# ChristianFeldmann/libHM

Hardware: AMD Instinct MI355X
Metric: decoded Mpixels/s (luma), 2160p Main10 reconstruction + loop filters (higher is better)
Workload: dtype int16 samples / int32 accumulate; 1 GPU; 3840x2160 Main10 lowdelay_P pictures, pre-parsed CTU metadata: prep+MC+dequant/IT/recon+deblock+SAO, batch of 16 independent pictures per step, inputs resident in HBM; sub_benchmark=full, streams=2, parallelism=frame-parallel, 1 process per GPU, no data-path collective

## Files before the change

libhm_amd/csrc/hmgpu_api.hip:

```cpp
#include "hmgpu_host.h"

#include <algorithm>
#include <cstdio>
#include <cstring>
#include <cstdlib>
#include <new>
#include <vector>

namespace hmgpu_host __attribute__((visibility("hidden"))) {

hipError_t h2d_small(hmgpu_ctx* c, void* dst, const void* src, size_t bytes, hipStream_t hs) {
  const size_t need = (bytes + 63) & ~(size_t)63;
  if (!c->bounce || need > hmgpu_ctx::kBounceSeg) return hipMemcpyAsync(dst, src, bytes, hipMemcpyHostToDevice, hs);
  if (c->bounce_off + need > hmgpu_ctx::kBounceSeg) {
    hipStream_t streams[3] = {c->stream, c->copy_stream, c->copy_stream2};
    for (int k = 0; k < 3; k++) (void)hipEventRecord(c->bounce_ev[c->bounce_seg][k], streams[k]);
    c->bounce_used[c->bounce_seg] = true;
    c->bounce_seg = (c->bounce_seg + 1) % hmgpu_ctx::kBounceSegs;
    c->bounce_off = 0;
    if (c->bounce_used[c->bounce_seg]) for (int k = 0; k < 3; k++) (void)hipEventSynchronize(c->bounce_ev[c->bounce_seg][k]);
  }
  char* at = c->bounce + (size_t)c->bounce_seg * hmgpu_ctx::kBounceSeg + c->bounce_off;
  memcpy(at, src, bytes);
  c->bounce_off += need;
// ... 224 lines not shown
  if (c->fmt != 1) {
    for (int i = 0; i < b.n; i++) {
      const PicDev& d = c->pics[b.pic[i]].dev;
      HIP_TRY(c, hipMemsetAsync(d.resid[1], 0, (size_t)((char*)d.resid[2] - (char*)d.resid[1]) + c->coef_elems[2] * sizeof(int16_t), c->stream));
    }
  }
  McArgs ma;
  memset(&ma, 0, sizeof(ma));
  ma.n = b.n; ma.width = c->seq.width; ma.height = c->seq.height; ma.log2ctu = c->seq.log2_ctu_size; ma.ctus_w = c->ctus_w;
  ma.tw = c->grid_w / 2; ma.npics = c->seq.max_pictures;
  ma.slab = c->plane_slab; ma.pic_stride = 2 * c->plane_bytes; ma.slab_bytes = ma.pic_stride * c->pics.size(); ma.sao_off = (uint32_t)c->plane_bytes;
  for (size_t i = 0; i < c->pics.size(); i++)
    if (c->pics[i].sao_applied) (i < 32 ? ma.sao_mask_lo : ma.sao_mask_hi) |= 1u << (i & 31);
  for (int i = 0; i < b.n; i++) {
    const PicDev& d = c->pics[b.pic[i]].dev;
    ma.first_ctu[i] = b.first_ctu[i]; ma.num_ctus[i] = b.num_ctus[i];
    ma.tmv[i] = d.tmv; ma.slices[i] = d.slices;
  }
  const PicDev& d0 = c->pics[b.pic[0]].dev;
  const char* const base0 = (const char*)c->pics[b.pic[0]].planes;
  uint32_t bps = (uint32_t)std::max(4, std::min(b.n >= 4 ? 12 : 24, max_ctus / 8 + 1));
  {
    ItxArgs ia;
    memset(&ia, 0, sizeof(ia));
    ia.n = b.n; ia.class_mask = 0xf;
    for (int k = 0; k < 3; k++) { ia.rtw[k] = (c->grid_w / 2) >> (k ? c->csx : 0); ia.bd[k] = d0.bd[k]; }
    ia.csx = c->csx; ia.csy = c->csy;
    for (int k = 0; k < 4; k++) ia.tu_cap[k] = c->tu_cap[k];
    for (int i = 0; i < b.n; i++) {
      const PicDev& d = c->pics[b.pic[i]].dev;
      for (int k = 0; k < 4; k++) ia.tu[i][k] = d.tu[k];
      ia.tu_count[i] = d.tu_count;
      for (int k = 0; k < 3; k++) { ia.coef[i][k] = d.coef[k]; ia.resid[i][k] = d.resid[k]; }
      ia.sl_m[i] = d.sl_m;
    }
    ProfScope ps(c, K_ITX);
    launch_itx(ia, bps, c->stream);
    bool any_ccp = false;
    for (int i = 0; i < b.n; i++) any_ccp |= c->pics[b.pic[i]].dev.ccp[0] != nullptr;
    if (any_ccp) launch_ccp(c->d_pics, b, max_ctus, c->stream);
  }
  {
    ProfScope ps(c, K_MC_LUMA);
    ma.pitch = c->pitch[0]; ma.bd = c->seq.bit_depth_luma;
    ma.origin_off = (uint32_t)((const char*)d0.rec[0] - base0);
    ma.rtw = c->grid_w / 2;
    for (int i = 0; i < b.n; i++) { ma.dst[i] = c->pics[b.pic[i]].dev.rec[0]; ma.resid[i] = c->pics[b.pic[i]].dev.resid[0]; }
    launch_mc_luma(ma, max_ctus, any_wp, any_bi, c->stream);
    if (any_cells) { ProfScope pc(c, K_MC_CELLS); launch_mc_luma_cells(c->d_pics, c->d_finals, b, max_ctus, c->seq.log2_ctu_size, any_wp, c->stream); }
  }
  if (c->fmt != 1) {
    ProfScope ps(c, K_MC_CHROMA);
    launch_mc_chroma_fmt(c->d_pics, c->d_finals, b, max_ctus, c->seq.log2_ctu_size, c->fmt, any_wp, c->stream);
  } else if (c->seq.chroma_format != 0) {
    ProfScope ps(c, K_MC_CHROMA);
    ma.pitch = c->pitch[1]; ma.bd = c->seq.bit_depth_chroma;
    ma.origin_off = (uint32_t)((const char*)d0.rec[1] - base0);
    ma.cr_off = 0;
    ma.rtw = c->grid_w / 4;
    for (int i = 0; i < b.n; i++) {
      const PicDev& d = c->pics[b.pic[i]].dev;
      ma.dst[i] = d.rec[1]; ma.dst2[i] = d.rec[2]; ma.resid[i] = d.resid[1]; ma.resid2[i] = d.resid[2];
    }
    launch_mc_chroma(ma, max_ctus, any_wp, any_bi, c->stream);
    if (any_cells) { ProfScope pc(c, K_MC_CELLS); launch_mc_chroma_cells(c->d_pics, c->d_finals, b, max_ctus, c->seq.log2_ctu_size, any_wp, c->stream); }
  }
  if (any_intra) {
    ProfScope ps(c, K_INTRA);
    launch_intra(c->d_pics, b, c->d_ctu_order, c->num_ctus, !any_islice, c->stream);
    if (c->fmt == 2) launch_intra_chroma_422(c->d_pics, b, c->stream);
    for (int i = 0; i < b.n; i++) if (std::find(c->intra_launched.begin(), c->intra_launched.end(), b.pic[i]) == c->intra_launched.end()) c->intra_launched.push_back(b.pic[i]);
  }
  HIP_TRY(c, hipGetLastError());
  return HMGPU_OK;
}

hmgpu_status run_filter(hmgpu_ctx* c, const Batch& b, int stages) {
// ... 129 lines not shown
  c->grid_w = c->ctus_w * c->pw; c->grid_h = c->ctus_h * c->pw;
  c->fmt = seq->chroma_format == 0 ? 1 : seq->chroma_format;
  c->csx = c->fmt == 3 ? 0 : 1; c->csy = c->fmt == 1 ? 1 : 0;
  c->mx[0] = 128; c->mx[1] = c->mx[2] = 128 >> c->csx;
  c->my[0] = 80; c->my[1] = c->my[2] = 80 >> c->csy;
  c->pitch[0] = (int)align_up((size_t)seq->width, 64) + 2 * c->mx[0] + 64;
  c->pitch[1] = c->pitch[2] = kCStep * ((int)align_up((size_t)seq->width >> c->csx, 64) + 2 * c->mx[1] + 64);
  c->rows[0] = c->ctus_h * c->ctu + 2 * c->my[0] + 8; c->rows[1] = c->rows[2] = ((c->ctus_h * c->ctu) >> c->csy) + 2 * c->my[1] + 8;
  c->coef_elems[0] = (size_t)c->num_ctus * c->ctu * c->ctu;
  c->coef_elems[1] = c->coef_elems[2] = c->coef_elems[0] >> (c->csx + c->csy);
  {
    const size_t blocks = ((size_t)c->num_ctus * (c->parts / 4) + 255) / 256;
    const size_t per_shard = (blocks + kTuShards - 1) / kTuShards;
    const uint32_t per_block[4] = {4 * 384, 4 * 96, 4 * 24, 4 * 4};
    for (int k = 0; k < 4; k++) c->tu_cap[k] = (uint32_t)(per_shard * (c->fmt == 1 ? per_block[k] : 3u * (1024u >> (2 * k))));
  }
  c->pics.resize(seq->max_pictures);
  c->h_finals.resize(seq->max_pictures);
  hmgpu_status st = HMGPU_OK;
  c->plane_bytes = plane_set_bytes(c);
  if (hipMalloc((void**)&c->plane_slab, c->plane_bytes * 2 * seq->max_pictures) != hipSuccess ||
      hipMemset(c->plane_slab, 0, c->plane_bytes * 2 * seq->max_pictures) != hipSuccess) st = HMGPU_EDEVICE;
  for (int i = 0; i < seq->max_pictures && st == HMGPU_OK; i++) st = alloc_picture(c, c->pics[i]);
  if (st == HMGPU_OK) {
    {
      std::vector<int32_t> order;
      for (int d = 0; d <= 2 * (c->ctus_h - 1) + c->ctus_w - 1; d++)
        for (int r = 0; r < c->ctus_h; r++) { const int col = d - 2 * r; if (col >= 0 && col < c->ctus_w) order.push_back(r * c->ctus_w + col); }
      if (hipMalloc((void**)&c->d_ctu_order, order.size() * sizeof(int32_t)) != hipSuccess ||
          hipMemcpy(c->d_ctu_order, order.data(), order.size() * sizeof(int32_t), hipMemcpyHostToDevice) != hipSuccess) st = HMGPU_EDEVICE;
// ... 429 lines not shown
```

libhm_amd/csrc/hmgpu_dev.h:

```cpp
#pragma once
#include <hip/hip_runtime.h>
#include <stdint.h>
#include "../../include/hmgpu.h"

namespace hmgpu {

constexpr int kMaxBatch = 16;
constexpr int kMaxPics = 64;
constexpr int kTuShards = 8;
constexpr int kCStep = 2;

struct __attribute__((aligned(16))) BlkInfo {
  int16_t mv[2][2];
  int8_t  ref[2];
  int8_t  qp;
  uint8_t flags;
  uint8_t edge;
  uint8_t log2cu;
  uint16_t slice;
};
static_assert(sizeof(BlkInfo) == 16, "BlkInfo must be 16 bytes");

enum : uint8_t {
  BF_VALID = 1,
// ... 105 lines not shown
  int32_t fmt, csx, csy;
  const int8_t* ccp[2];
  uint8_t* ctu_intra;
  uint32_t* intra_done;
  uint32_t* fault;
  int32_t debug_skip_ctu;
};

struct Batch {
  int32_t n;
  int32_t pic[kMaxBatch];
  int32_t first_ctu[kMaxBatch];
  int32_t num_ctus[kMaxBatch];
};

struct McArgs {
  int32_t n, mode, log2n, per;
  int32_t width, height, log2ctu, ctus_w;
  int32_t tw, pitch, bd, npics;
  int32_t first_ctu[kMaxBatch], num_ctus[kMaxBatch];
  const TileMv* tmv[kMaxBatch];
  int16_t* dst[kMaxBatch];
  int16_t* dst2[kMaxBatch];
  const int16_t* resid[kMaxBatch];
  const int16_t* resid2[kMaxBatch];
  int32_t rtw, pad_;
  const SliceDev* slices[kMaxBatch];
  const char* slab;
  uint64_t pic_stride, slab_bytes;
  uint32_t sao_off, origin_off, cr_off;
  uint32_t sao_mask_lo, sao_mask_hi;
};

struct ItxArgs {
  int32_t n; uint32_t class_mask;
  int32_t blocks[4];
  int32_t rtw[3], bd[3];
  int32_t csx, csy;
  uint32_t tu_cap[4];
  const TuRec* tu[kMaxBatch][4];
  const uint32_t* tu_count[kMaxBatch];
  const int16_t* coef[kMaxBatch][3];
  int16_t* resid[kMaxBatch][3];
  const uint8_t* sl_m[kMaxBatch];
};

#define HMGPU_AS1 __attribute__((address_space(1)))
// ... 204 lines not shown
```

libhm_amd/csrc/k_itx.hip:

```cpp
#include "hmgpu_dev.h"
#include "itx_core.h"
#include <algorithm>

namespace hmgpu {

template <int LOG2N> struct ItxLds {
  static constexpr int BYTES = PkCfg<LOG2N>::TPB * PkCfg<LOG2N>::TU_ELEMS * 2;
};
constexpr int kItxLdsBytes = std::max(std::max(ItxLds<2>::BYTES, ItxLds<3>::BYTES), std::max(ItxLds<4>::BYTES, ItxLds<5>::BYTES));

struct ItxPic {
  const TuRec* list; uint32_t count_cap; const uint32_t* count;
  const int16_t* coef[3]; int16_t* resid[3]; int32_t rtw[3], bd[3]; const uint8_t* sl_m;
  int32_t csx, csy;
};
template <typename T> __device__ inline T by_comp(const T (&v)[3], int comp) { return comp == 0 ? v[0] : comp == 1 ? v[1] : v[2]; }

template <int LOG2N>
__device__ inline void itx_class(const ItxPic& P, int bx, int nbx, char* __restrict__ lds_raw) {
  constexpr int N = 1 << LOG2N;
  const TuRec* __restrict__ list = P.list;
  const uint32_t cap = P.count_cap;
  const int j = threadIdx.x / N, n = threadIdx.x % N;
  int16_t* buf = reinterpret_cast<int16_t*>(lds_raw) + j * PkCfg<LOG2N>::TU_ELEMS;
  constexpr int TPW = 64 / N;
  const int jw = (threadIdx.x & 63) / N;
  const uint32_t stride = (uint32_t)nbx * 4 * TPW;
  uint32_t t = ((uint32_t)bx * 4 + (threadIdx.x >> 6)) * TPW + jw;
  struct Rec { uint32_t w0, w1, w2; };
  auto load_rec = [&](uint32_t ti, Rec& r) {
    r.w0 = r.w1 = r.w2 = 0;
    if (ti < cap) { const uint32_t* rp = reinterpret_cast<const uint32_t*>(list + ti); r.w0 = ldg(rp); r.w1 = ldg(rp + 1); r.w2 = ldg(rp + 2); }
  };
  Rec rc, rn;
  load_rec(t, rc);
  load_rec(t + stride, rn);
  const uint32_t count = min(ldg(P.count), cap);
  auto load_levels = [&](uint32_t ti, const Rec& r, uint32_t (&lv)[N / 2]) {
#pragma unroll
    for (int i = 0; i < N / 2; i++) lv[i] = 0;
    if (ti < count) {
      const int16_t* lev = by_comp(P.coef, r.w1 & 3) + r.w2 + n * N;
      if constexpr (N == 4) { const u32x2 a = ldg2(lev); lv[0] = a.x; lv[1] = a.y; }
      else {
#pragma unroll
        for (int i = 0; i < N / 8; i++) { const u32x4 a = ldg4(lev + i * 8); lv[4 * i] = a.x; lv[4 * i + 1] = a.y; lv[4 * i + 2] = a.z; lv[4 * i + 3] = a.w; }
      }
// ... 114 lines not shown
```

libhm_amd/csrc/k_mc.hip:

```cpp
#include "mc_core.h"
#include "itx_core.h"
#include <type_traits>

namespace hmgpu {

typedef u32x4 u32x4_a4 __attribute__((aligned(4)));
#if defined(MC_EXP) && (MC_EXP & 1)
__device__ inline u32x4 ldg4_a4(const void* p) { const uint32_t v = (uint32_t)(uintptr_t)p; return u32x4{v, v + 1, v + 2, v + 3}; }
#elif defined(MC_NT)
__device__ inline u32x4 ldg4_a4(const void* p) { return __builtin_nontemporal_load((const u32x4_a4 HMGPU_AS1*)p); }
#else
__device__ inline u32x4 ldg4_a4(const void* p) { return *(const u32x4_a4 HMGPU_AS1*)p; }
#endif
#ifndef MC_LB_LUMA
#define MC_LB_LUMA 7
#endif
#ifndef MC_LB_CHROMA
#define MC_LB_CHROMA 8
#endif

__device__ inline uint32_t pk_sub(uint32_t a, uint32_t b) {
  return __builtin_bit_cast(uint32_t, __builtin_bit_cast(short2v, a) - __builtin_bit_cast(short2v, b));
}

// ... 48 lines not shown
  asm("v_ashrrev_i32_sdwa %0, %1, %2 dst_sel:WORD_1 dst_unused:UNUSED_PRESERVE src0_sel:DWORD src1_sel:DWORD" : "+v"(d) : "v"(sh), "v"(hi));
  return d;
}

template <bool CHROMA> struct McLds {
  static constexpr int ROW_DW = CHROMA ? 128 : 256;
  struct { uint32_t body[2 * ROW_DW], halo[2 * ROW_DW]; } w[4];
  uint32_t taps[144];
  uint32_t htap[CHROMA ? 36 : 1];
#ifdef MC_LDS_PAD
  uint32_t pad[MC_LDS_PAD / 4];
#endif
};

struct Square { int sx, sy, ext; };
__device__ inline bool square_of_block(const McArgs& a, int& slot, Square& g) {
  int lb;
  if (a.mode) { slot = blockIdx.x & (a.n - 1); lb = (int)(blockIdx.x >> a.log2n) * a.per + (int)blockIdx.y; }
  else { slot = blockIdx.x; lb = blockIdx.y; }
  if (lb >= a.num_ctus[slot]) return false;
  const int ctu = a.first_ctu[slot] + lb, ctu_sz = 1 << a.log2ctu;
  g.sx = (ctu % a.ctus_w) * ctu_sz; g.sy = (ctu / a.ctus_w) * ctu_sz; g.ext = min(ctu_sz, 64);
  return true;
}

struct WpTile { bool active; int w0, o0, w1, o1, log2wd; };
template <bool WP>
__device__ inline WpTile wp_tile(const SliceDev* __restrict__ slices, uint32_t flags, uint32_t wpw, int comp) {
  WpTile w = {false, 1, 0, 1, 0, 0};
  if constexpr (WP) {
    const SliceDev& sd = slices[wpw >> 16];
    w.active = ldg(&sd.weighted_pred) != 0;
    if (w.active) {
      w.log2wd = ldg(&sd.wp_log2_denom[comp ? 1 : 0]);
      const int l0 = (flags & TM_FIRST_L1) ? 1 : 0, r0 = wpw & 15, r1 = (wpw >> 4) & 15;
      w.w0 = ldg(&sd.wp_weight[l0][r0][comp]); w.o0 = ldg(&sd.wp_offset[l0][r0][comp]);
      if (flags & TM_BI) { w.w1 = ldg(&sd.wp_weight[1][r1][comp]); w.o1 = ldg(&sd.wp_offset[1][r1][comp]); }
// ... 62 lines not shown
      const auto sw = __builtin_amdgcn_permlane32_swap(res[0][j], res[1][j], false, false);
      o[2 * j] = __builtin_amdgcn_perm(sw[1], sw[0], 0x05040100u);
      o[2 * j + 1] = __builtin_amdgcn_perm(sw[1], sw[0], 0x07060302u);
    }
    stg4(dst, u32x4{o[0], o[1], o[2], o[3]});
    return;
  }
#pragma unroll
  for (int r = 0; r < 2; r++) {
    int16_t* row = dst + (ptrdiff_t)r * pitch;
    if constexpr (W == 8) { u32x4 v = {res[r][0], res[r][1], res[r][2], res[r][3]}; stg4(row, v); }
    else { u32x2 v = {res[r][0], res[r][1]}; stg2(row, v); }
  }
}

__device__ inline u32x4 load_tile_rec(const McArgs& a, int slot, const Square& g, int x, int y) {
  const bool tin = x < g.sx + g.ext && y < g.sy + g.ext && x < a.width && y < a.height;
  u32x4 tm = {0, 0, 0, 0};
  if (tin) tm = ldg4(a.tmv[slot] + (size_t)(y >> 3) * a.tw + (x >> 3));
  return tm;
}
__device__ inline bool tile_is_top(const u32x4 tm, int r, int partner_lane) {
  const uint32_t u0 = __shfl((int)tm.x, partner_lane), u1 = __shfl((int)tm.y, partner_lane), u2 = __shfl((int)tm.z, partner_lane);
  return r == 0 || !(u0 == tm.x && u1 == tm.y && u2 == tm.z);
}

constexpr uint32_t kWinLimit = 0xffff0000u;
constexpr uint32_t kResidLimit = 0x7fffff00u;
template <bool BUF> struct Win;
template <> struct Win<true> {
  typedef uint32_t ref;
  __amdgpu_buffer_rsrc_t rs;
  uint32_t stride;
  __device__ inline Win(const McArgs& a, int) : rs(__builtin_amdgcn_make_buffer_rsrc((void*)a.slab, 0, kWinLimit, 0x00020000)), stride((uint32_t)a.pic_stride) {}
  __device__ inline ref nowhere() const { return kWinLimit; }
  __device__ inline ref plane(const McArgs& a, int pic) const {
    const uint32_t m = pic & 32 ? a.sao_mask_hi : a.sao_mask_lo;
    return (uint32_t)pic * stride + (__builtin_amdgcn_ubfe(m, (uint32_t)pic & 31u, 1u) ? a.sao_off : 0u) + a.origin_off;
  }
  __device__ inline ref at(ref pl, int row, int pitch, int x) const { return pl + (uint32_t)((row * pitch + x) * 2); }
  __device__ inline u32x4 load(ref o) const { return __builtin_bit_cast(u32x4, __builtin_amdgcn_raw_buffer_load_b128(rs, o, 0, 0)); }
};
template <> struct Win<false> {
  typedef const char* ref;
  const char* dummy;
  __device__ inline Win(const McArgs& a, int slot) : dummy(reinterpret_cast<const char*>(a.tmv[slot])) {}
  __device__ inline ref nowhere() const { return dummy; }
  __device__ inline ref plane(const McArgs& a, int pic) const {
    const uint32_t m = pic & 32 ? a.sao_mask_hi : a.sao_mask_lo;
    return a.slab + (size_t)(uint32_t)pic * a.pic_stride + (__builtin_amdgcn_ubfe(m, (uint32_t)pic & 31u, 1u) ? a.sao_off : 0u) + a.origin_off;
  }
  __device__ inline ref at(ref pl, int row, int pitch, int x) const { return pl + ((ptrdiff_t)row * pitch + x) * 2; }
  __device__ inline u32x4 load(ref p) const { return ldg4_a4(p); }
};

__device__ inline uint32_t from_right(uint32_t own, uint32_t first, bool take) {
  const uint32_t t = (uint32_t)__builtin_amdgcn_update_dpp(0, (int)first, 0x101, 0xf, 0xf, true);
  return take ? t : own;
}
__device__ inline u32x4 from_right(const u32x4 own, const u32x4 first, bool take) {
  return u32x4{from_right(own.x, first.x, take), from_right(own.y, first.y, take), from_right(own.z, first.z, take), from_right(own.w, first.w, take)};
}

__device__ inline void h_item_luma(const u32x4 (&r)[4], const uint32_t* __restrict__ tap, int sh1, uint32_t* __restrict__ out) {
// ... 34 lines not shown
__device__ inline uint32_t low_half(uint32_t v, int lane) { return (uint32_t)__shfl((int)v, lane & 31); }
__device__ inline const char* low_half(const char* p, int lane) {
  const uint64_t v = (uint64_t)(uintptr_t)p;
  return (const char*)(uintptr_t)(((uint64_t)low_half((uint32_t)(v >> 32), lane) << 32) | low_half((uint32_t)v, lane));
}

#ifndef MC_NO_F0
#define MC_F0 1
#endif
#ifndef MC_NO_R15
#define MC_R15 1
#endif
template <bool WP, bool BI, bool BUF>
__global__ void __launch_bounds__(256, (WP || BI) ? 1 : MC_LB_LUMA) k_mc_luma(const McArgs a) {
  __shared__ __attribute__((aligned(16))) McLds<false> S;
  int slot; Square g;
  if (!square_of_block(a, slot, g)) return;
  const int tid = threadIdx.x, lane = tid & 63, wave = tid >> 6;
  if (wave * 16 >= g.ext) return;
  const int pitch = a.pitch, bd = a.bd;
  const int tx = lane & 7, q = (lane >> 3) & 3, r = lane >> 5;
  const int x0 = g.sx + tx * 8, y0 = g.sy + wave * 16 + r * 8;
  const u32x4 tm = load_tile_rec(a, slot, g, x0, y0);
  if (lane < 36) *reinterpret_cast<u32x4*>(&S.taps[4 * lane]) = ldg4(&g_taps_luma.e[0][0] + 4 * lane);
  const uint32_t flags = tm.z >> 24, rmask = (tm.w >> 8) & 0xff;
  const bool active = (flags & TM_ACTIVE) != 0;
  if (!__ballot(active)) return;
#if defined(MC_EXP) && (MC_EXP & 64)
  bool top = tile_is_top(tm, r, lane ^ 32);
  if (wave > 0) {
    const u32x4 up = load_tile_rec(a, slot, g, x0, y0 - 8);
    if (r == 0 && up.x == tm.x && up.y == tm.y && up.z == tm.z) top = false;
  }
#else
  const bool top = tile_is_top(tm, r, lane ^ 32);
#endif
#ifdef MC_DEDUP
  const bool same_right = tx < 7 && !tile_is_top(tm, 1, lane + 1);
#else
  const bool same_right = false;
#endif
  const bool any_bi = BI && __ballot((flags & TM_BI) != 0) != 0;
  wave_lds_sync();
#ifdef MC_LDS_PAD
  if (a.n < 0) S.pad[tid] = 1;
#endif
  const int npass = any_bi ? 2 : 1;
  const int head = bd >= 12 ? 2 : 14 - bd;
  const int sh1 = 6 - head;
  uint32_t* const body_t = &S.w[wave].body[r * 256 + tx * 2];
  uint32_t* const halo_t = &S.w[wave].halo[r * 256 + tx * 2];
  const Win<BUF> win(a, slot);
  typedef typename Win<BUF>::ref wref;
  const wref nowhere = win.nowhere();
  WpTile wp = {false, 1, 0, 1, 0, 0};
  if constexpr (WP) wp = wp_tile<WP>(a.slices[slot], flags, tm.w, 0);
  uint32_t rsd[2][4];
  {
    const uint32_t qm = active ? (rmask >> (q & 2)) & 3 : 0u;
    const __amdgpu_buffer_rsrc_t rr = __builtin_amdgcn_make_buffer_rsrc((void*)a.resid[slot], 0, kResidLimit, 0x00020000);
    const uint32_t ro = qm ? (uint32_t)((((y0 >> 3) * a.rtw + (x0 >> 3)) * 64 + q * 8) * 2) : kResidLimit;
    const u32x4 r0 = __builtin_bit_cast(u32x4, __builtin_amdgcn_raw_buffer_load_b128(rr, ro, 0, 0));
    const u32x4 r1 = __builtin_bit_cast(u32x4, __builtin_amdgcn_raw_buffer_load_b128(rr, ro + 64, 0, 0));
    rsd[0][0] = qm & 1 ? r0.x : 0u; rsd[0][1] = qm & 1 ? r0.y : 0u; rsd[1][0] = qm & 1 ? r1.x : 0u; rsd[1][1] = qm & 1 ? r1.y : 0u;
    rsd[0][2] = qm & 2 ? r0.z : 0u; rsd[0][3] = qm & 2 ? r0.w : 0u; rsd[1][2] = qm & 2 ? r1.z : 0u; rsd[1][3] = qm & 2 ? r1.w : 0u;
  }
  uint32_t park[8];
#pragma unroll
  for (int x = 0; x < 8; x++) park[x] = 0;
#pragma unroll 1
  for (int pass = 0; pass < npass; pass++) {
    const bool bact = active && (pass == 0 || (flags & TM_BI));
    const uint32_t mv = pass ? tm.y : tm.x;
    const uint32_t fr = (tm.z >> (4 * pass)) & 15;
#ifdef MC_F0
    const bool yz = (fr & 12) == 0, xz = (fr & 3) == 0;
#else
    const bool yz = false, xz = false;
#endif
    const bool ptop = top || yz;
    const bool bon = bact && (!yz || q < 2), hon = bact && ptop && (!yz || q >= 2);
    const int xs = x0 + (int)(int16_t)(mv & 0xffff) - (xz ? 0 : 3);
    const bool two = !xz || (xs & 1);
    const uint32_t* const tap = &S.taps[((xz ? 4u : (fr & 3)) * 2 + (xs & 1)) * 12];
    const wref pw = win.at(win.plane(a, (int)((tm.z >> (8 + 8 * pass)) & (kMaxPics - 1))), y0 + ((int)mv >> 16) - (yz ? 4 : 3) + 2 * q, pitch, xs & ~1);
    const uint32_t vidx = yz ? 5u : (fr >> 2) & 3;
    const uint64_t bon_m = __ballot(bon), hon_m = __ballot(hon);
#ifdef MC_R15
    const bool b2on = bon && (q != 3 || (r == 0 && !((__ballot(ptop) >> (lane + 32)) & 1)));
#else
    const bool b2on = bon;
#endif
    const uint64_t b2on_m = __ballot(b2on);
    const bool rb_shared = same_right && ((bon_m >> (lane + 1)) & 1), rb2_shared = same_right && ((b2on_m >> (lane + 1)) & 1);
    const bool rh_shared = same_right && ((hon_m >> (lane + 1)) & 1);
    auto h_phase = [&](auto with_halo) {
      constexpr bool HALO = decltype(with_halo)::value;
      u32x4 rb[4], rh[4];
      {
        const wref p0 = bon ? pw + pitch * 16 : nowhere, p1 = bon && two && !rb_shared ? p0 + 16 : nowhere;
// ... 55 lines not shown
      for (int j = 0; j < 5; j++) {
        const int gp = q + j;
        const uint32_t* src = gp < 4 ? above + gp * 16 : body_t + (gp - 4) * 16;
        uint32_t pr[8];
#pragma unroll
        for (int c = 0; c < 4; c++) { const u32x2 v = *reinterpret_cast<const u32x2*>(src + c * 64); pr[2 * c] = v.x; pr[2 * c + 1] = v.y; }
#pragma unroll
        for (int x = 0; x < 8; x++) {
          if (j == 0) { v6[0][x] = dot2_seed(pr[x], A[0], seed); v6[1][x] = dot2_seed(pr[x], B[0], seed); }
          else {
            if (j < 4) v6[0][x] = dot2(pr[x], A[j], v6[0][x]);
            v6[1][x] = dot2(pr[x], B[j], v6[1][x]);
          }
        }
      }
      finish_rows<8, WP, BI>(v6, park, pass, (flags & TM_BI) != 0, bd, wp, rsd, a.dst[slot] + (ptrdiff_t)(y0 + 2 * q) * pitch + x0, pitch);
    }
    if (BI && pass + 1 < npass) wave_lds_sync();
  }
}

struct alignas(16) HTapsChroma { uint32_t e[9][4]; };
constexpr HTapsChroma make_htaps_chroma() {
  constexpr int c[9][4] = {{0, 64, 0, 0}, {-2, 58, 10, -2}, {-4, 54, 16, -2}, {-6, 46, 28, -4}, {-4, 36, 36, -4}, {-4, 28, 46, -6}, {-2, 16, 54, -4}, {-2, 10, 58, -2},
                           {64, 0, 0, 0}};
  HTapsChroma t = {};
  for (int f = 0; f < 9; f++)
    for (int k = 0; k < 4; k++) t.e[f][k] = pk16(c[f][k] / 2, c[f][k] / 2);
  return t;
}
__device__ const HTapsChroma g_htaps_chroma = make_htaps_chroma();
// ... 50 lines not shown
#pragma unroll
      for (int k = 1; k < 4; k++) v = pk_mad(d[x + k], tc[k], v);
      h[row][x] = sh1 == 0 ? pk_shl(v, 0x00010001u) : pk_ashr(v, (uint32_t)(sh1 - 1) * 0x10001u);
    }
  }
#pragma unroll
  for (int c = 0; c < 2; c++) {
    *reinterpret_cast<u32x2*>(out + c * 32) = u32x2{__builtin_amdgcn_perm(h[1][2 * c], h[0][2 * c], 0x05040100u), __builtin_amdgcn_perm(h[1][2 * c + 1], h[0][2 * c + 1], 0x05040100u)};
    *reinterpret_cast<u32x2*>(out + 64 + c * 32) = u32x2{__builtin_amdgcn_perm(h[1][2 * c], h[0][2 * c], 0x07060302u), __builtin_amdgcn_perm(h[1][2 * c + 1], h[0][2 * c + 1], 0x07060302u)};
  }
}

template <bool WP, bool BI, bool BUF>
__global__ void __launch_bounds__(256, (WP && BI) ? 6 : MC_LB_CHROMA) k_mc_chroma(const McArgs a) {
  __shared__ __attribute__((aligned(16))) McLds<true> S;
  int slot; Square g;
  if (!square_of_block(a, slot, g)) return;
  const int tid = threadIdx.x, lane = tid & 63, wave = tid >> 6;
  if (wave * 16 >= g.ext) return;
  const int pitch = a.pitch, bd = a.bd;
  const int tx = lane & 7, hq = (lane >> 3) & 1, r = (lane >> 4) & 1, hi = lane >> 5;
  const int x0 = g.sx + tx * 8, y0 = g.sy + wave * 16 + r * 8;
  const u32x4 tm = load_tile_rec(a, slot, g, x0, y0);
  if (lane < 36) *reinterpret_cast<u32x4*>(&S.taps[4 * lane]) = ldg4(&g_taps_chroma.e[0][0] + 4 * lane);
  else if (lane < 45) *reinterpret_cast<u32x4*>(&S.htap[4 * (lane - 36)]) = ldg4(&g_htaps_chroma.e[0][0] + 4 * (lane - 36));
  const uint32_t flags = tm.z >> 24, rmask = (tm.w >> 8) & 0xff;
  const bool active = (flags & TM_ACTIVE) != 0;
  if (!__ballot(active)) return;
  const bool top = tile_is_top(tm, r, lane ^ 16);
  const bool any_bi = BI && __ballot((flags & TM_BI) != 0) != 0;
  wave_lds_sync();
  const int npass = any_bi ? 2 : 1;
  const int head = bd >= 12 ? 2 : 14 - bd;
  const int sh1 = 6 - head;
  uint32_t* const hout = (hi ? S.w[wave].halo : S.w[wave].body) + r * 128 + tx * 2 + hq * 16;
  uint32_t* const body_v = &S.w[wave].body[r * 128 + hi * 64 + tx * 2];
  uint32_t* const halo_v = &S.w[wave].halo[r * 128 + hi * 64 + tx * 2];
  WpTile wp = {false, 1, 0, 1, 0, 0};
  if constexpr (WP) wp = wp_tile<WP>(a.slices[slot], flags, tm.w, 1 + hi);
  uint32_t rsd[2][2];
  {
    const bool coded = active && (rmask & (hi ? TR_CR : TR_CB));
    const int xc = x0 >> 1, yc = (y0 >> 1) + 2 * hq;
    const __amdgpu_buffer_rsrc_t rr = __builtin_amdgcn_make_buffer_rsrc((void*)a.resid[slot], 0, kResidLimit, 0x00020000);
    const uint32_t ro = coded ? (uint32_t)(((((yc >> 3) * a.rtw + (xc >> 3)) * 8 + resid_slot(yc)) * 8 + (xc & 4)) * 2) + (hi ? (uint32_t)((const char*)a.resid2[slot] - (const char*)a.resid[slot]) : 0u) : kResidLimit;
    const u32x2 r0 = __builtin_bit_cast(u32x2, __builtin_amdgcn_raw_buffer_load_b64(rr, ro, 0, 0));
    const u32x2 r1 = __builtin_bit_cast(u32x2, __builtin_amdgcn_raw_buffer_load_b64(rr, ro + 64, 0, 0));
    rsd[0][0] = coded ? r0.x : 0u; rsd[0][1] = coded ? r0.y : 0u; rsd[1][0] = coded ? r1.x : 0u; rsd[1][1] = coded ? r1.y : 0u;
  }
  uint32_t park[4] = {0, 0, 0, 0};
  const Win<BUF> win(a, slot);
  typedef typename Win<BUF>::ref wref;
#pragma unroll 1
  for (int pass = 0; pass < npass; pass++) {
    const bool vact = active && (pass == 0 || (flags & TM_BI));
    const uint32_t mv = pass ? tm.y : tm.x, fr = (tm.z >> (4 * pass)) & 15;
    const int ix = (int)(int16_t)(mv & 0xffff), iy = (int)mv >> 16;
    const int yf = ((iy & 1) << 2) | ((fr >> 2) & 3);
#ifdef MC_F0
    const bool yz = yf == 0;
#else
    const bool yz = false;
#endif
    const bool ptop = top || yz;
    const bool hact = vact && (hi == 0 ? (!yz || hq == 0) : (ptop && (!yz || hq == 1)));
#ifdef MC_R15
    const bool row2 = hi != 0 || hq == 0 || (r == 0 && !((__ballot(ptop) >> (lane | 16)) & 1));
#else
    const bool row2 = true;
#endif
    if (hact) {
      const int xf = ((ix & 1) << 2) | (fr & 3);
#ifdef MC_F0
      const bool xz = xf == 0;
#else
      const bool xz = false;
#endif
      const int xs = (x0 >> 1) + (ix >> 1) - (xz ? 0 : 1), ys = (y0 >> 1) + (iy >> 1) - (yz ? 2 : 1) + (hi ? 0 : 4) + 2 * hq;
      const wref p0 = win.at(win.plane(a, (int)((tm.z >> (8 + 8 * pass)) & (kMaxPics - 1))), ys, pitch, kCStep * xs);
      const int rowb = pitch * 2;
      u32x4 rr[4];
#if defined(MC_CEXP) && (MC_CEXP & 1)
      const bool ld = hi == 0;
#elif defined(MC_CEXP) && (MC_CEXP & 2)
      const bool ld = false;
#else
      const bool ld = true;
#endif
      rr[0] = win.load(ld ? p0 : win.nowhere()); rr[1] = win.load(ld && !xz ? p0 + 16 : win.nowhere());
      rr[2] = win.load(ld && row2 ? p0 + rowb : win.nowhere()); rr[3] = win.load(ld && row2 && !xz ? p0 + rowb + 16 : win.nowhere());
      h_item_chroma(rr, &S.htap[(xz ? 8 : xf) * 4], sh1, hout);
    }
    wave_lds_sync();
    if (vact) {
// ... 8 lines not shown
      for (int j = 0; j < 3; j++) {
        const int gp = hq + j;
        const uint32_t* src = gp < 2 ? above + gp * 16 : body_v + (gp - 2) * 16;
        const u32x2 c0 = *reinterpret_cast<const u32x2*>(src), c1 = *reinterpret_cast<const u32x2*>(src + 32);
        const uint32_t pr[4] = {c0.x, c0.y, c1.x, c1.y};
#pragma unroll
        for (int x = 0; x < 4; x++) {
          if (j == 0) { v6[0][x] = dot2_seed(pr[x], A[0], seed); v6[1][x] = dot2_seed(pr[x], B[0], seed); }
          else {
            if (j < 2) v6[0][x] = dot2(pr[x], A[j], v6[0][x]);
            v6[1][x] = dot2(pr[x], B[j], v6[1][x]);
          }
        }
      }
      const int xc = x0 >> 1, yc = (y0 >> 1) + 2 * hq;
      finish_rows<4, WP, BI, true>(v6, park, pass, (flags & TM_BI) != 0, bd, wp, rsd, a.dst[slot] + (ptrdiff_t)(yc + hi) * pitch + kCStep * xc, pitch);
    }
    if (BI && pass + 1 < npass) wave_lds_sync();
  }
}

template <typename K>
static void launch_mc(K kernel, McArgs& a, int max_ctus, hipStream_t s) {
  a.mode = 0; a.log2n = 0; a.per = 0;
  dim3 grid((unsigned)a.n, (unsigned)max_ctus);
  if (a.n <= 8 && (8 % a.n) == 0) {
    const int m = 8 / a.n;
    a.mode = 1; a.per = (max_ctus + m - 1) / m;
    while ((1 << a.log2n) < a.n) a.log2n++;
    grid = dim3(8u, (unsigned)a.per);
  }
// ... 28 lines not shown
```

Baseline: 188,400 Mpixels/s.

## Regroup MC kernel args into per-slot structs loaded as scalars in prologue

Splits McArgs into a shared geometry block and 64-byte-aligned per-picture slots, so each MC block can fetch its slot's pointers with one contiguous scalar load and keep them in SGPRs through asm pins and sched barriers. The itx TU record load becomes a single bounds-checked buffer b96 load, and the chroma tap table copy is merged into one predicated loop. A host check also rejects configurations whose TU capacity would overflow the 32-bit buffer range. The aim is less kernel-argument indexing overhead and fewer VGPR and scalar instructions in the prologue, at the cost of a layout rigidly tied to static_asserts.

```diff
diff --git a/libhm_amd/csrc/hmgpu_api.hip b/libhm_amd/csrc/hmgpu_api.hip
--- a/libhm_amd/csrc/hmgpu_api.hip
+++ b/libhm_amd/csrc/hmgpu_api.hip
@@ -262,8 +262,8 @@
     if (c->pics[i].sao_applied) (i < 32 ? ma.sao_mask_lo : ma.sao_mask_hi) |= 1u << (i & 31);
   for (int i = 0; i < b.n; i++) {
     const PicDev& d = c->pics[b.pic[i]].dev;
-    ma.first_ctu[i] = b.first_ctu[i]; ma.num_ctus[i] = b.num_ctus[i];
-    ma.tmv[i] = d.tmv; ma.slices[i] = d.slices;
+    ma.s[i].first_ctu = b.first_ctu[i]; ma.s[i].num_ctus = b.num_ctus[i];
+    ma.s[i].tmv = d.tmv; ma.s[i].slices = d.slices;
   }
   const PicDev& d0 = c->pics[b.pic[0]].dev;
   const char* const base0 = (const char*)c->pics[b.pic[0]].planes;
@@ -293,7 +293,7 @@
     ma.pitch = c->pitch[0]; ma.bd = c->seq.bit_depth_luma;
     ma.origin_off = (uint32_t)((const char*)d0.rec[0] - base0);
     ma.rtw = c->grid_w / 2;
-    for (int i = 0; i < b.n; i++) { ma.dst[i] = c->pics[b.pic[i]].dev.rec[0]; ma.resid[i] = c->pics[b.pic[i]].dev.resid[0]; }
+    for (int i = 0; i < b.n; i++) { ma.s[i].dst = c->pics[b.pic[i]].dev.rec[0]; ma.s[i].resid = c->pics[b.pic[i]].dev.resid[0]; }
     launch_mc_luma(ma, max_ctus, any_wp, any_bi, c->stream);
     if (any_cells) { ProfScope pc(c, K_MC_CELLS); launch_mc_luma_cells(c->d_pics, c->d_finals, b, max_ctus, c->seq.log2_ctu_size, any_wp, c->stream); }
   }
@@ -308,7 +308,7 @@
     ma.rtw = c->grid_w / 4;
     for (int i = 0; i < b.n; i++) {
       const PicDev& d = c->pics[b.pic[i]].dev;
-      ma.dst[i] = d.rec[1]; ma.dst2[i] = d.rec[2]; ma.resid[i] = d.resid[1]; ma.resid2[i] = d.resid[2];
+      ma.s[i].dst = d.rec[1]; ma.s[i].dst2 = d.rec[2]; ma.s[i].resid = d.resid[1]; ma.s[i].resid2 = d.resid[2];
     }
     launch_mc_chroma(ma, max_ctus, any_wp, any_bi, c->stream);
     if (any_cells) { ProfScope pc(c, K_MC_CELLS); launch_mc_chroma_cells(c->d_pics, c->d_finals, b, max_ctus, c->seq.log2_ctu_size, any_wp, c->stream); }
@@ -468,6 +468,8 @@
     const size_t per_shard = (blocks + kTuShards - 1) / kTuShards;
     const uint32_t per_block[4] = {4 * 384, 4 * 96, 4 * 24, 4 * 4};
     for (int k = 0; k < 4; k++) c->tu_cap[k] = (uint32_t)(per_shard * (c->fmt == 1 ? per_block[k] : 3u * (1024u >> (2 * k))));
+    for (int k = 0; k < 4; k++)
+      if (per_shard * (c->fmt == 1 ? per_block[k] : 3u * (1024u >> (2 * k))) * sizeof(TuRec) > 0xffffffffull) { hmgpu_destroy(c); return HMGPU_EUNSUPPORTED; }
   }
   c->pics.resize(seq->max_pictures);
   c->h_finals.resize(seq->max_pictures);
diff --git a/libhm_amd/csrc/hmgpu_dev.h b/libhm_amd/csrc/hmgpu_dev.h
--- a/libhm_amd/csrc/hmgpu_dev.h
+++ b/libhm_amd/csrc/hmgpu_dev.h
@@ -143,23 +143,27 @@
   int32_t num_ctus[kMaxBatch];
 };
 
-struct McArgs {
+struct McGeo {
   int32_t n, mode, log2n, per;
   int32_t width, height, log2ctu, ctus_w;
   int32_t tw, pitch, bd, npics;
-  int32_t first_ctu[kMaxBatch], num_ctus[kMaxBatch];
-  const TileMv* tmv[kMaxBatch];
-  int16_t* dst[kMaxBatch];
-  int16_t* dst2[kMaxBatch];
-  const int16_t* resid[kMaxBatch];
-  const int16_t* resid2[kMaxBatch];
-  int32_t rtw, pad_;
-  const SliceDev* slices[kMaxBatch];
+  int32_t rtw;
+  uint32_t sao_off, origin_off, cr_off;
+  uint32_t sao_mask_lo, sao_mask_hi;
   const char* slab;
   uint64_t pic_stride, slab_bytes;
-  uint32_t sao_off, origin_off, cr_off;
-  uint32_t sao_mask_lo, sao_mask_hi;
-};
+};
+struct alignas(64) McSlot {
+  const TileMv* tmv;
+  int16_t* dst;
+  int16_t* dst2;
+  const int16_t* resid;
+  const int16_t* resid2;
+  const SliceDev* slices;
+  int32_t first_ctu, num_ctus;
+};
+struct McArgs : McGeo { McSlot s[kMaxBatch]; };
+static_assert(sizeof(McGeo) == 96 && sizeof(McSlot) == 64 && sizeof(McArgs) == 128 + 64 * kMaxBatch, "McArgs: the layout k_mc.hip's scalar loads are written for");
 
 struct ItxArgs {
   int32_t n; uint32_t class_mask;
diff --git a/libhm_amd/csrc/k_itx.hip b/libhm_amd/csrc/k_itx.hip
--- a/libhm_amd/csrc/k_itx.hip
+++ b/libhm_amd/csrc/k_itx.hip
@@ -28,9 +28,10 @@
   const uint32_t stride = (uint32_t)nbx * 4 * TPW;
   uint32_t t = ((uint32_t)bx * 4 + (threadIdx.x >> 6)) * TPW + jw;
   struct Rec { uint32_t w0, w1, w2; };
+  const __amdgpu_buffer_rsrc_t lrs = __builtin_amdgcn_make_buffer_rsrc((void*)list, 0, cap * 12u, 0x00020000);
   auto load_rec = [&](uint32_t ti, Rec& r) {
-    r.w0 = r.w1 = r.w2 = 0;
-    if (ti < cap) { const uint32_t* rp = reinterpret_cast<const uint32_t*>(list + ti); r.w0 = ldg(rp); r.w1 = ldg(rp + 1); r.w2 = ldg(rp + 2); }
+    const auto v = __builtin_amdgcn_raw_buffer_load_b96(lrs, min(ti, cap) * 12u, 0, 0);
+    r.w0 = (uint32_t)v[0]; r.w1 = (uint32_t)v[1]; r.w2 = (uint32_t)v[2];
   };
   Rec rc, rn;
   load_rec(t, rc);
diff --git a/libhm_amd/csrc/k_mc.hip b/libhm_amd/csrc/k_mc.hip
--- a/libhm_amd/csrc/k_mc.hip
+++ b/libhm_amd/csrc/k_mc.hip
@@ -86,13 +86,27 @@
 };
 
 struct Square { int sx, sy, ext; };
-__device__ inline bool square_of_block(const McArgs& a, int& slot, Square& g) {
-  int lb;
-  if (a.mode) { slot = blockIdx.x & (a.n - 1); lb = (int)(blockIdx.x >> a.log2n) * a.per + (int)blockIdx.y; }
-  else { slot = blockIdx.x; lb = blockIdx.y; }
-  if (lb >= a.num_ctus[slot]) return false;
-  const int ctu = a.first_ctu[slot] + lb, ctu_sz = 1 << a.log2ctu;
-  g.sx = (ctu % a.ctus_w) * ctu_sz; g.sy = (ctu / a.ctus_w) * ctu_sz; g.ext = min(ctu_sz, 64);
+__device__ inline void pin_scalars(McGeo& G) {
+  asm volatile("" : "+s"(G.n), "+s"(G.mode), "+s"(G.log2n), "+s"(G.per), "+s"(G.width), "+s"(G.height), "+s"(G.log2ctu), "+s"(G.ctus_w),
+                    "+s"(G.tw), "+s"(G.pitch), "+s"(G.bd), "+s"(G.npics));
+  asm volatile("" : "+s"(G.rtw), "+s"(G.sao_off), "+s"(G.origin_off), "+s"(G.cr_off), "+s"(G.sao_mask_lo), "+s"(G.sao_mask_hi), "+s"(G.slab),
+                    "+s"(G.pic_stride));
+}
+__device__ inline void pin_scalars(McSlot& P) {
+  asm volatile("" : "+s"(P.tmv), "+s"(P.dst), "+s"(P.dst2), "+s"(P.resid), "+s"(P.resid2), "+s"(P.slices), "+s"(P.first_ctu), "+s"(P.num_ctus));
+}
+__device__ inline bool mc_prologue(const McArgs& a, McGeo& G, McSlot& P, Square& g) {
+  G = a;
+  pin_scalars(G);
+  __builtin_amdgcn_sched_barrier(0);
+  const int bx = (int)blockIdx.x, by = (int)blockIdx.y;
+  const int slot = G.mode ? bx & (G.n - 1) : bx, lb = G.mode ? (bx >> G.log2n) * G.per + by : by;
+  P = a.s[slot];
+  pin_scalars(P);
+  __builtin_amdgcn_sched_barrier(0);
+  if (lb >= P.num_ctus) return false;
+  const int ctu = P.first_ctu + lb, ctu_sz = 1 << G.log2ctu;
+  g.sx = (ctu % G.ctus_w) * ctu_sz; g.sy = (ctu / G.ctus_w) * ctu_sz; g.ext = min(ctu_sz, 64);
   return true;
 }
 
@@ -185,10 +199,10 @@
   }
 }
 
-__device__ inline u32x4 load_tile_rec(const McArgs& a, int slot, const Square& g, int x, int y) {
-  const bool tin = x < g.sx + g.ext && y < g.sy + g.ext && x < a.width && y < a.height;
+__device__ inline u32x4 load_tile_rec(const McGeo& G, const McSlot& P, const Square& g, int x, int y) {
+  const bool tin = x < g.sx + g.ext && y < g.sy + g.ext && x < G.width && y < G.height;
   u32x4 tm = {0, 0, 0, 0};
-  if (tin) tm = ldg4(a.tmv[slot] + (size_t)(y >> 3) * a.tw + (x >> 3));
+  if (tin) tm = ldg4(P.tmv + (size_t)(y >> 3) * G.tw + (x >> 3));
   return tm;
 }
 __device__ inline bool tile_is_top(const u32x4 tm, int r, int partner_lane) {
@@ -196,6 +210,7 @@
   return r == 0 || !(u0 == tm.x && u1 == tm.y && u2 == tm.z);
 }
 
+__device__ inline uint32_t sao_mask_of(const McGeo& a, int pic) { return pic & 32 ? a.sao_mask_hi : a.sao_mask_lo; }
 constexpr uint32_t kWinLimit = 0xffff0000u;
 constexpr uint32_t kResidLimit = 0x7fffff00u;
 template <bool BUF> struct Win;
@@ -203,10 +218,10 @@
   typedef uint32_t ref;
   __amdgpu_buffer_rsrc_t rs;
   uint32_t stride;
-  __device__ inline Win(const McArgs& a, int) : rs(__builtin_amdgcn_make_buffer_rsrc((void*)a.slab, 0, kWinLimit, 0x00020000)), stride((uint32_t)a.pic_stride) {}
+  __device__ inline Win(const McGeo& a, const McSlot&) : rs(__builtin_amdgcn_make_buffer_rsrc((void*)a.slab, 0, kWinLimit, 0x00020000)), stride((uint32_t)a.pic_stride) {}
   __device__ inline ref nowhere() const { return kWinLimit; }
-  __device__ inline ref plane(const McArgs& a, int pic) const {
-    const uint32_t m = pic & 32 ? a.sao_mask_hi : a.sao_mask_lo;
+  __device__ inline ref plane(const McGeo& a, int pic) const {
+    const uint32_t m = sao_mask_of(a, pic);
     return (uint32_t)pic * stride + (__builtin_amdgcn_ubfe(m, (uint32_t)pic & 31u, 1u) ? a.sao_off : 0u) + a.origin_off;
   }
   __device__ inline ref at(ref pl, int row, int pitch, int x) const { return pl + (uint32_t)((row * pitch + x) * 2); }
@@ -215,10 +230,10 @@
 template <> struct Win<false> {
   typedef const char* ref;
   const char* dummy;
-  __device__ inline Win(const McArgs& a, int slot) : dummy(reinterpret_cast<const char*>(a.tmv[slot])) {}
+  __device__ inline Win(const McGeo&, const McSlot& P) : dummy(reinterpret_cast<const char*>(P.tmv)) {}
   __device__ inline ref nowhere() const { return dummy; }
-  __device__ inline ref plane(const McArgs& a, int pic) const {
-    const uint32_t m = pic & 32 ? a.sao_mask_hi : a.sao_mask_lo;
+  __device__ inline ref plane(const McGeo& a, int pic) const {
+    const uint32_t m = sao_mask_of(a, pic);
     return a.slab + (size_t)(uint32_t)pic * a.pic_stride + (__builtin_amdgcn_ubfe(m, (uint32_t)pic & 31u, 1u) ? a.sao_off : 0u) + a.origin_off;
   }
   __device__ inline ref at(ref pl, int row, int pitch, int x) const { return pl + ((ptrdiff_t)row * pitch + x) * 2; }
@@ -283,14 +298,14 @@
 template <bool WP, bool BI, bool BUF>
 __global__ void __launch_bounds__(256, (WP || BI) ? 1 : MC_LB_LUMA) k_mc_luma(const McArgs a) {
   __shared__ __attribute__((aligned(16))) McLds<false> S;
-  int slot; Square g;
-  if (!square_of_block(a, slot, g)) return;
+  McGeo G; McSlot P; Square g;
+  if (!mc_prologue(a, G, P, g)) return;
   const int tid = threadIdx.x, lane = tid & 63, wave = tid >> 6;
   if (wave * 16 >= g.ext) return;
-  const int pitch = a.pitch, bd = a.bd;
+  const int pitch = G.pitch, bd = G.bd;
   const int tx = lane & 7, q = (lane >> 3) & 3, r = lane >> 5;
   const int x0 = g.sx + tx * 8, y0 = g.sy + wave * 16 + r * 8;
-  const u32x4 tm = load_tile_rec(a, slot, g, x0, y0);
+  const u32x4 tm = load_tile_rec(G, P, g, x0, y0);
   if (lane < 36) *reinterpret_cast<u32x4*>(&S.taps[4 * lane]) = ldg4(&g_taps_luma.e[0][0] + 4 * lane);
   const uint32_t flags = tm.z >> 24, rmask = (tm.w >> 8) & 0xff;
   const bool active = (flags & TM_ACTIVE) != 0;
@@ -298,7 +313,7 @@
 #if defined(MC_EXP) && (MC_EXP & 64)
   bool top = tile_is_top(tm, r, lane ^ 32);
   if (wave > 0) {
-    const u32x4 up = load_tile_rec(a, slot, g, x0, y0 - 8);
+    const u32x4 up = load_tile_rec(G, P, g, x0, y0 - 8);
     if (r == 0 && up.x == tm.x && up.y == tm.y && up.z == tm.z) top = false;
   }
 #else
@@ -312,23 +327,23 @@
   const bool any_bi = BI && __ballot((flags & TM_BI) != 0) != 0;
   wave_lds_sync();
 #ifdef MC_LDS_PAD
-  if (a.n < 0) S.pad[tid] = 1;
+  if (G.n < 0) S.pad[tid] = 1;
 #endif
   const int npass = any_bi ? 2 : 1;
   const int head = bd >= 12 ? 2 : 14 - bd;
   const int sh1 = 6 - head;
   uint32_t* const body_t = &S.w[wave].body[r * 256 + tx * 2];
   uint32_t* const halo_t = &S.w[wave].halo[r * 256 + tx * 2];
-  const Win<BUF> win(a, slot);
+  const Win<BUF> win(G, P);
   typedef typename Win<BUF>::ref wref;
   const wref nowhere = win.nowhere();
   WpTile wp = {false, 1, 0, 1, 0, 0};
-  if constexpr (WP) wp = wp_tile<WP>(a.slices[slot], flags, tm.w, 0);
+  if constexpr (WP) wp = wp_tile<WP>(P.slices, flags, tm.w, 0);
   uint32_t rsd[2][4];
   {
     const uint32_t qm = active ? (rmask >> (q & 2)) & 3 : 0u;
-    const __amdgpu_buffer_rsrc_t rr = __builtin_amdgcn_make_buffer_rsrc((void*)a.resid[slot], 0, kResidLimit, 0x00020000);
-    const uint32_t ro = qm ? (uint32_t)((((y0 >> 3) * a.rtw + (x0 >> 3)) * 64 + q * 8) * 2) : kResidLimit;
+    const __amdgpu_buffer_rsrc_t rr = __builtin_amdgcn_make_buffer_rsrc((void*)P.resid, 0, kResidLimit, 0x00020000);
+    const uint32_t ro = qm ? (uint32_t)((((y0 >> 3) * G.rtw + (x0 >> 3)) * 64 + q * 8) * 2) : kResidLimit;
     const u32x4 r0 = __builtin_bit_cast(u32x4, __builtin_amdgcn_raw_buffer_load_b128(rr, ro, 0, 0));
     const u32x4 r1 = __builtin_bit_cast(u32x4, __builtin_amdgcn_raw_buffer_load_b128(rr, ro + 64, 0, 0));
     rsd[0][0] = qm & 1 ? r0.x : 0u; rsd[0][1] = qm & 1 ? r0.y : 0u; rsd[1][0] = qm & 1 ? r1.x : 0u; rsd[1][1] = qm & 1 ? r1.y : 0u;
@@ -352,7 +367,7 @@
     const int xs = x0 + (int)(int16_t)(mv & 0xffff) - (xz ? 0 : 3);
     const bool two = !xz || (xs & 1);
     const uint32_t* const tap = &S.taps[((xz ? 4u : (fr & 3)) * 2 + (xs & 1)) * 12];
-    const wref pw = win.at(win.plane(a, (int)((tm.z >> (8 + 8 * pass)) & (kMaxPics - 1))), y0 + ((int)mv >> 16) - (yz ? 4 : 3) + 2 * q, pitch, xs & ~1);
+    const wref pw = win.at(win.plane(G, (int)((tm.z >> (8 + 8 * pass)) & (kMaxPics - 1))), y0 + ((int)mv >> 16) - (yz ? 4 : 3) + 2 * q, pitch, xs & ~1);
     const uint32_t vidx = yz ? 5u : (fr >> 2) & 3;
     const uint64_t bon_m = __ballot(bon), hon_m = __ballot(hon);
 #ifdef MC_R15
@@ -438,7 +453,7 @@
           }
         }
       }
-      finish_rows<8, WP, BI>(v6, park, pass, (flags & TM_BI) != 0, bd, wp, rsd, a.dst[slot] + (ptrdiff_t)(y0 + 2 * q) * pitch + x0, pitch);
+      finish_rows<8, WP, BI>(v6, park, pass, (flags & TM_BI) != 0, bd, wp, rsd, P.dst + (ptrdiff_t)(y0 + 2 * q) * pitch + x0, pitch);
     }
     if (BI && pass + 1 < npass) wave_lds_sync();
   }
@@ -519,16 +534,16 @@
 template <bool WP, bool BI, bool BUF>
 __global__ void __launch_bounds__(256, (WP && BI) ? 6 : MC_LB_CHROMA) k_mc_chroma(const McArgs a) {
   __shared__ __attribute__((aligned(16))) McLds<true> S;
-  int slot; Square g;
-  if (!square_of_block(a, slot, g)) return;
+  McGeo G; McSlot P; Square g;
+  if (!mc_prologue(a, G, P, g)) return;
   const int tid = threadIdx.x, lane = tid & 63, wave = tid >> 6;
   if (wave * 16 >= g.ext) return;
-  const int pitch = a.pitch, bd = a.bd;
+  const int pitch = G.pitch, bd = G.bd;
   const int tx = lane & 7, hq = (lane >> 3) & 1, r = (lane >> 4) & 1, hi = lane >> 5;
   const int x0 = g.sx + tx * 8, y0 = g.sy + wave * 16 + r * 8;
-  const u32x4 tm = load_tile_rec(a, slot, g, x0, y0);
-  if (lane < 36) *reinterpret_cast<u32x4*>(&S.taps[4 * lane]) = ldg4(&g_taps_chroma.e[0][0] + 4 * lane);
-  else if (lane < 45) *reinterpret_cast<u32x4*>(&S.htap[4 * (lane - 36)]) = ldg4(&g_htaps_chroma.e[0][0] + 4 * (lane - 36));
+  const u32x4 tm = load_tile_rec(G, P, g, x0, y0);
+  static_assert(offsetof(McLds<true>, htap) == offsetof(McLds<true>, taps) + 36 * 16, "the tap tables are copied as one piece");
+  if (lane < 45) *reinterpret_cast<u32x4*>(&S.taps[4 * lane]) = ldg4(lane < 36 ? &g_taps_chroma.e[0][0] + 4 * lane : &g_htaps_chroma.e[0][0] + 4 * (lane - 36));
   const uint32_t flags = tm.z >> 24, rmask = (tm.w >> 8) & 0xff;
   const bool active = (flags & TM_ACTIVE) != 0;
   if (!__ballot(active)) return;
@@ -542,19 +557,19 @@
   uint32_t* const body_v = &S.w[wave].body[r * 128 + hi * 64 + tx * 2];
   uint32_t* const halo_v = &S.w[wave].halo[r * 128 + hi * 64 + tx * 2];
   WpTile wp = {false, 1, 0, 1, 0, 0};
-  if constexpr (WP) wp = wp_tile<WP>(a.slices[slot], flags, tm.w, 1 + hi);
+  if constexpr (WP) wp = wp_tile<WP>(P.slices, flags, tm.w, 1 + hi);
   uint32_t rsd[2][2];
   {
     const bool coded = active && (rmask & (hi ? TR_CR : TR_CB));
     const int xc = x0 >> 1, yc = (y0 >> 1) + 2 * hq;
-    const __amdgpu_buffer_rsrc_t rr = __builtin_amdgcn_make_buffer_rsrc((void*)a.resid[slot], 0, kResidLimit, 0x00020000);
-    const uint32_t ro = coded ? (uint32_t)(((((yc >> 3) * a.rtw + (xc >> 3)) * 8 + resid_slot(yc)) * 8 + (xc & 4)) * 2) + (hi ? (uint32_t)((const char*)a.resid2[slot] - (const char*)a.resid[slot]) : 0u) : kResidLimit;
+    const __amdgpu_buffer_rsrc_t rr = __builtin_amdgcn_make_buffer_rsrc((void*)P.resid, 0, kResidLimit, 0x00020000);
+    const uint32_t ro = coded ? (uint32_t)(((((yc >> 3) * G.rtw + (xc >> 3)) * 8 + resid_slot(yc)) * 8 + (xc & 4)) * 2) + (hi ? (uint32_t)((const char*)P.resid2 - (const char*)P.resid) : 0u) : kResidLimit;
     const u32x2 r0 = __builtin_bit_cast(u32x2, __builtin_amdgcn_raw_buffer_load_b64(rr, ro, 0, 0));
     const u32x2 r1 = __builtin_bit_cast(u32x2, __builtin_amdgcn_raw_buffer_load_b64(rr, ro + 64, 0, 0));
     rsd[0][0] = coded ? r0.x : 0u; rsd[0][1] = coded ? r0.y : 0u; rsd[1][0] = coded ? r1.x : 0u; rsd[1][1] = coded ? r1.y : 0u;
   }
   uint32_t park[4] = {0, 0, 0, 0};
-  const Win<BUF> win(a, slot);
+  const Win<BUF> win(G, P);
   typedef typename Win<BUF>::ref wref;
 #pragma unroll 1
   for (int pass = 0; pass < npass; pass++) {
@@ -582,7 +597,7 @@
       const bool xz = false;
 #endif
       const int xs = (x0 >> 1) + (ix >> 1) - (xz ? 0 : 1), ys = (y0 >> 1) + (iy >> 1) - (yz ? 2 : 1) + (hi ? 0 : 4) + 2 * hq;
-      const wref p0 = win.at(win.plane(a, (int)((tm.z >> (8 + 8 * pass)) & (kMaxPics - 1))), ys, pitch, kCStep * xs);
+      const wref p0 = win.at(win.plane(G, (int)((tm.z >> (8 + 8 * pass)) & (kMaxPics - 1))), ys, pitch, kCStep * xs);
       const int rowb = pitch * 2;
       u32x4 rr[4];
 #if defined(MC_CEXP) && (MC_CEXP & 1)
@@ -621,7 +636,7 @@
         }
       }
       const int xc = x0 >> 1, yc = (y0 >> 1) + 2 * hq;
-      finish_rows<4, WP, BI, true>(v6, park, pass, (flags & TM_BI) != 0, bd, wp, rsd, a.dst[slot] + (ptrdiff_t)(yc + hi) * pitch + kCStep * xc, pitch);
+      finish_rows<4, WP, BI, true>(v6, park, pass, (flags & TM_BI) != 0, bd, wp, rsd, P.dst + (ptrdiff_t)(yc + hi) * pitch + kCStep * xc, pitch);
     }
     if (BI && pass + 1 < npass) wave_lds_sync();
   }
```

Measured after the change: 193,000 Mpixels/s, median of 5. 1.02x the previous value.
